# squellww/super-resolution-system

Measured on AMD Instinct MI355X. Metric: megapixels/sec tile+blend+QA at 200MP, 1/2/4/8 GPU, higher is better.
Workload: dtype f32; 1 GPU; 720p->200MP 17320x11550 canvas, 25 tiles 4124x2970, 6-level Laplacian blend (cosine weights) + PSNR + SSIM(uniform7,gauss11,simple); tile_pixels=306207000, canvas_pixels=200046000, parallelism=single, stream=assessment of image i on a second HIP stream beside tile+pyramids of image i+1

## Files before the change

include/sr_hip.h:

```cpp
#ifndef SR_HIP_H
#define SR_HIP_H

#include <stddef.h>
#include <stdint.h>

#ifdef __cplusplus
extern "C" {
#endif

#define SR_API __attribute__((visibility("default")))

enum sr_status {
    SR_OK = 0,
    SR_ERR_INVALID_ARG = -1,
    SR_ERR_SHAPE = -2,
    SR_ERR_OOM = -3,
    SR_ERR_HIP = -4,
    SR_ERR_COMM = -5,
    SR_ERR_UNSUPPORTED = -6
};

enum sr_pad_mode { SR_PAD_MIRROR = 0, SR_PAD_REPLICATE = 1, SR_PAD_REFLECT = 2, SR_PAD_CONSTANT = 3 };
enum sr_weight_type { SR_W_LINEAR = 0, SR_W_COSINE = 1, SR_W_SIGMOID = 2,
                      SR_W_ONES = 3 };
// ... 212 lines not shown
    double ssim_simple;
} sr_assess_sums;
SR_API int sr_assess_u8_async(sr_ctx *ctx, const uint8_t *d_a, int64_t stride_a, const uint8_t *d_b,
                              int64_t stride_b, int h, int w, int cn, int gray_shift, double data_range,
                              int row_begin, int row_end, int flags, sr_assess_sums *d_out);
SR_API int sr_assess_u8(sr_ctx *ctx, const uint8_t *d_a, int64_t stride_a, const uint8_t *d_b,
                        int64_t stride_b, int h, int w, int cn, int gray_shift, double data_range,
                        int row_begin, int row_end, int flags, sr_assess_sums *h_out);
SR_API int sr_assess_resized_u8_async(sr_ctx *ctx, const uint8_t *d_a, int64_t stride_a, const uint8_t *d_b,
                                      int64_t stride_b, int h, int w, int cn, int dst_h, int dst_w,
                                      int gray_shift, double data_range, int flags, sr_assess_sums *d_out);
SR_API int sr_assess_resized_u8(sr_ctx *ctx, const uint8_t *d_a, int64_t stride_a, const uint8_t *d_b,
                                int64_t stride_b, int h, int w, int cn, int dst_h, int dst_w, int gray_shift,
                                double data_range, int flags, sr_assess_sums *h_out);
SR_API int sr_ssim_count(int h, int w, int mode, int row_begin, int row_end, uint64_t *count);
typedef struct sr_quality_cell {
    uint64_t sse;
    double ssim_uniform;
    double ssim_gauss;
    double ssim_simple;
} sr_quality_cell;
SR_API int sr_quality_map_u8(sr_ctx *ctx, const uint8_t *d_a, int64_t stride_a, const uint8_t *d_b, int64_t stride_b,
                             int h, int w, int cn, int gray_shift, double data_range, const int *h_xedges, int gw,
                             const int *h_yedges, int gh, int flags, sr_quality_cell *h_out);
SR_API int sr_quality_map_counts(int h, int w, int mode, const int *h_xedges, int gw, const int *h_yedges, int gh,
                                 uint64_t *counts);
typedef struct sr_ms_ssim_level {
    double sum_lcs;
    double sum_cs;
    uint64_t count;
// ... 381 lines not shown
```

super-resolution-system_amd/_native.py:

```python
from __future__ import annotations

import ctypes as C
import math
import os
import threading
from typing import List, Optional, Sequence, Tuple

import numpy as np

_HERE = os.path.dirname(os.path.abspath(__file__))
LIB_PATH = os.environ.get("SR_LIB_PATH") or os.path.join(_HERE, "libsrhip.so")

SR_OK = 0
SR_ERR_INVALID_ARG, SR_ERR_SHAPE, SR_ERR_OOM, SR_ERR_HIP, SR_ERR_COMM, SR_ERR_UNSUPPORTED = -1, -2, -3, -4, -5, -6
PAD_MODES = {"mirror": 0, "replicate": 1, "reflect": 2, "constant": 3}
WEIGHT_TYPES = {"linear": 0, "cosine": 1, "sigmoid": 2, "ones": 3}
SSIM_MODES = {"uniform": 0, "gauss": 1, "simple": 2}
SR_U8, SR_F32, SR_F64 = 0, 1, 2
POISSON_MAX_SIDE = 16385


class SrNativeError(RuntimeError):
    """HIP / library failure (SR_ERR_HIP, SR_ERR_OOM, SR_ERR_COMM, SR_ERR_UNSUPPORTED)."""

# ... 238 lines not shown
    "sr_sse_u8": (_i, [_vp, _vp, _i64, _vp, _i64, _i, _i64, C.POINTER(C.c_uint64)]),
    "sr_sse_u8_async": (_i, [_vp, _vp, _i64, _vp, _i64, _i, _i64, _vp]),
    "sr_psnr_from_sse": (_dbl, [C.c_uint64, C.c_uint64, _dbl]),
    "sr_seam_scan": (_i, [_vp, _vp, _i64, _i, _i, _i, C.POINTER(TileRect), C.POINTER(_vp), C.POINTER(_i64), _i, _i, _i, _i,
                          _dbl, C.POINTER(SeamRecord), _i, _pi]),
    "sr_sse_f32": (_i, [_vp, _vp, _i64, _vp, _i64, _i, _i64, C.POINTER(_dbl)]),
    "sr_weighted_blend_custom": (_i, [_vp, _i, C.POINTER(_vp), C.POINTER(_i64), C.POINTER(_vp), C.POINTER(_i64), _vp, _i64, _vp]),
    "sr_ssim_u8": (_i, [_vp, _vp, _i64, _vp, _i64, _i, _i, _i, _i, _i, _dbl, _i, _i, C.POINTER(_dbl), C.POINTER(C.c_uint64)]),
    "sr_ssim_float": (_i, [_vp, _i, _vp, _i64, _vp, _i64, _i, _i, _i, _i, _dbl, _i, _i, C.POINTER(_dbl), C.POINTER(C.c_uint64)]),
    "sr_ssim_u8_async": (_i, [_vp, _vp, _i64, _vp, _i64, _i, _i, _i, _i, _i, _dbl, _i, _i, _vp, C.POINTER(C.c_uint64)]),
    "sr_assess_u8_async": (_i, [_vp, _vp, _i64, _vp, _i64, _i, _i, _i, _i, _dbl, _i, _i, _i, _vp]),
    "sr_assess_u8": (_i, [_vp, _vp, _i64, _vp, _i64, _i, _i, _i, _i, _dbl, _i, _i, _i, C.POINTER(AssessSums)]),
    "sr_assess_resized_u8_async": (_i, [_vp, _vp, _i64, _vp, _i64, _i, _i, _i, _i, _i, _i, _dbl, _i, _vp]),
    "sr_assess_resized_u8": (_i, [_vp, _vp, _i64, _vp, _i64, _i, _i, _i, _i, _i, _i, _dbl, _i, C.POINTER(AssessSums)]),
    "sr_ssim_count": (_i, [_i, _i, _i, _i, _i, C.POINTER(C.c_uint64)]),
    "sr_quality_map_u8": (_i, [_vp, _vp, _i64, _vp, _i64, _i, _i, _i, _i, _dbl, _pi, _i, _pi, _i, _i, C.POINTER(QualityCell)]),
    "sr_quality_map_counts": (_i, [_i, _i, _i, _pi, _i, _pi, _i, C.POINTER(C.c_uint64)]),
    "sr_ms_ssim_plan": (_i, [_i, _i, _i, _pi, _pi, C.POINTER(C.c_uint64), C.POINTER(_sz)]),
    "sr_ms_ssim_u8": (_i, [_vp, _vp, _i64, _vp, _i64, _i, _i, _i, _i, _dbl, _i, C.POINTER(MsSsimLevel)]),
    "sr_ms_ssim_value": (_dbl, [C.POINTER(MsSsimLevel), _i, C.POINTER(_dbl)]),
    "sr_ms_ssim_planes": (_i, [_vp, _i, _vp, _vp]),
    "sr_bench_plan": (_i, [_i, _i, _i, _i, _i, _pi, _pi, C.POINTER(C.c_uint64), C.POINTER(C.c_uint64), C.POINTER(_sz)]),
    "sr_bench_u8": (_i, [_vp, _vp, _i64, _vp, _i64, _i, _i, _i, _i, _i, _dbl, C.POINTER(BenchSums)]),
    "sr_vif_plan": (_i, [_i, _i, _i, _i, _i, _pi, _pi, C.POINTER(C.c_uint64), C.POINTER(_sz)]),
    "sr_vif_window": (_i, [_i, C.POINTER(_dbl)]),
    "sr_vif_u8": (_i, [_vp, _vp, _i64, _vp, _i64, _i, _i, _i, _i, _i, C.POINTER(VifScale)]),
    "sr_vif_value": (_dbl, [C.POINTER(VifScale), _i]),
    "sr_gmsd_plan": (_i, [_i, _i, _i, _i, _i, _pi, _pi, C.POINTER(C.c_uint64), C.POINTER(_sz)]),
    "sr_gmsd_u8": (_i, [_vp, _vp, _i64, _vp, _i64, _i, _i, _i, _i, _i, C.POINTER(GmsdSums)]),
    "sr_gmsd_value": (_dbl, [C.POINTER(GmsdSums)]),
# ... 329 lines not shown


def color_table_class(glut: np.ndarray, terms: int = 64) -> int:
    g = np.ascontiguousarray(glut, dtype=np.float32).reshape(-1, 256)
    cls = C.c_int(-1)
    check(load().sr_color_table_class(g.ctypes.data_as(C.POINTER(C.c_float)), int(g.shape[0]), int(terms), C.byref(cls)))
    return cls.value


def ssim_count(h: int, w: int, mode: str, row_begin: int = 0, row_end: Optional[int] = None) -> int:
    n = C.c_uint64(0)
    check(load().sr_ssim_count(h, w, SSIM_MODES[mode], row_begin, h if row_end is None else row_end, C.byref(n)))
    return n.value


def _edge_array(edges, name: str):
    e = np.asarray(edges)
    if e.ndim != 1 or e.size < 2 or e.dtype.kind not in "iu":
        raise ValueError(f"{name}: need a flat list of at least two integer edges")
    if e.min() < -2 ** 31 or e.max() >= 2 ** 31:
        raise ValueError(f"{name}: edge out of range")
    return (C.c_int * e.size)(*[int(v) for v in e]), int(e.size) - 1


def quality_map_counts(h: int, w: int, mode: str, x_edges, y_edges) -> np.ndarray:
    xe, gw = _edge_array(x_edges, "x_edges")
    ye, gh = _edge_array(y_edges, "y_edges")
    out = np.zeros((gh, gw), dtype=np.uint64)
    check(load().sr_quality_map_counts(int(h), int(w), SSIM_MODES[mode], xe, gw, ye, gh,
                                       out.ctypes.data_as(C.POINTER(C.c_uint64))))
# ... 2187 lines not shown
```

super-resolution-system_amd/csrc/sr_assess.hip:

```cpp
#include <hip/hip_runtime.h>

#include <algorithm>
#include <cmath>
#include <cstdlib>
#include <cstring>
#include <mutex>
#include <set>
#include <vector>

#include "sr_ctx.h"
#include "sr_device.h"
#include "sr_ssim11.h"

__device__ __forceinline__ unsigned long long wave_sum_u64(unsigned long long v)
{
#pragma unroll
    for (int o = 32; o > 0; o >>= 1) v += __shfl_down(v, o, 64);
    return v;
}

__device__ __forceinline__ double wave_sum_f64(double v)
{
#pragma unroll
    for (int o = 32; o > 0; o >>= 1) v += __shfl_down(v, o, 64);
    return v;
}

__global__ __launch_bounds__(256) void k_sse_flat(const uint4 *__restrict__ a, const uint4 *__restrict__ b,
                                                  size_t nvec, const unsigned char *__restrict__ ta,
                                                  const unsigned char *__restrict__ tb, int ntail,
                                                  unsigned long long *__restrict__ out)
{
    unsigned long long s = 0;
    const size_t stride = (size_t)gridDim.x * blockDim.x;
    for (size_t i = (size_t)blockIdx.x * blockDim.x + threadIdx.x; i < nvec; i += stride) {
        const uint4 va = a[i], vb = b[i];
        const unsigned int wa[4] = {va.x, va.y, va.z, va.w}, wb[4] = {vb.x, vb.y, vb.z, vb.w};
        unsigned int p = 0;
#pragma unroll
        for (int k = 0; k < 4; ++k)
#pragma unroll
            for (int j = 0; j < 4; ++j) {
// ... 68 lines not shown
{
    const int x = blockIdx.x * 64 + threadIdx.x, y = blockIdx.y * 4 + threadIdx.y;
    if (x >= w || y >= h) return;
    gray[(size_t)y * gstride + x] = (unsigned char)gray_of(rgb + (size_t)y * stride + (size_t)x * 3, 3, shift);
}

struct CubicTab {
    int ofs;
    short c[4];
};

enum { ASSESS_SSE = 1, ASSESS_UNIFORM = 2, ASSESS_GAUSS = 4, ASSESS_SIMPLE = 8, ASSESS_ALL_BITS = 15 };

struct AssessParams {
    int h, w, shift, ry0, ry1, flags, same_c;
    int nch, ty;
    double c1a, c2a;
    double c1b, c2b;
    double k1u, k2u;
    double k[6];
};

template <int CN>
__device__ __forceinline__ void load_gray_pair(const unsigned char *__restrict__ a, long long sa,
                                               const unsigned char *__restrict__ b, long long sb, int sy, int sx,
                                               int shift, int &ga, int &gb, unsigned &sq)
{
    const unsigned char *pa = a + (size_t)sy * sa + (size_t)sx * CN;
    const unsigned char *pb = b + (size_t)sy * sb + (size_t)sx * CN;
    gray_pair<CN>(pa, pb, shift, ga, gb, sq);
}


__device__ __forceinline__ double fast_recip(double d)
{
// ... 50 lines not shown
        for (int c = 0; c < CN; ++c) {
            const int hs = v[0][c] * X.c[0] + v[1][c] * X.c[1] + v[2][c] * X.c[2] + v[3][c] * X.c[3];
            acc[c] += hs * (int)yc[ky];
        }
    }
#pragma unroll
    for (int c = 0; c < CN; ++c) {
        const int t = (acc[c] + (1 << 21)) >> 22;
        out[c] = t < 0 ? 0 : (t > 255 ? 255 : t);
    }
}

template <int CN>
__device__ __forceinline__ unsigned assess_load_chunk(const unsigned char *__restrict__ a, long long sa,
                                                      const unsigned char *__restrict__ b, long long sb,
                                                      const AssessParams &P, int bx0, int by0, int ch,
                                                      int rows_needed, unsigned (*XY)[AM_GP],
                                                      unsigned (*QQ)[AM_GP], unsigned (*PP)[AM_GP])
{
    unsigned sse = 0;
    const bool want_sse = (P.flags & ASSESS_SSE) != 0;
    for (int i = threadIdx.x; i < AM_CH * (AM_GP / 4); i += AM_TX) {
        const int ly = i / (AM_GP / 4), lx = (i - ly * (AM_GP / 4)) * 4;
        const int lr = ch * AM_CH + ly;
        if (lr >= rows_needed) break;
        const int gy = by0 - AM_R + lr, gx = bx0 - AM_R + lx;
        const int sy = reflect101(gy, P.h);
        int ga[4], gb[4];
        unsigned sq[4];
        if (gx >= 0 && gx + 3 < P.w) {
            const unsigned char *pa = a + (size_t)sy * sa + (size_t)gx * CN;
            const unsigned char *pb = b + (size_t)sy * sb + (size_t)gx * CN;
            if (CN == 3) {
                const u3_t qa = ld_u3_a1(pa), qb = ld_u3_a1(pb);
                const unsigned wa[3] = {qa.x, qa.y, qa.z}, wb[3] = {qb.x, qb.y, qb.z};
                int ca[12], cb[12];
#pragma unroll
// ... 24 lines not shown
        }
        u4_t vxy, vq, vp;
        unsigned txy[4], tq[4], tp[4];
#pragma unroll
        for (int k = 0; k < 4; ++k) {
            txy[k] = (unsigned)ga[k] | ((unsigned)gb[k] << 14);
            tq[k] = (unsigned)__mul24(ga[k], gb[k]);
            tp[k] = (unsigned)(__mul24(ga[k], ga[k]) + __mul24(gb[k], gb[k]));
        }
        vxy.x = txy[0]; vxy.y = txy[1]; vxy.z = txy[2]; vxy.w = txy[3];
        vq.x = tq[0]; vq.y = tq[1]; vq.z = tq[2]; vq.w = tq[3];
        vp.x = tp[0]; vp.y = tp[1]; vp.z = tp[2]; vp.w = tp[3];
        *(u4_t *)&XY[ly][lx] = vxy;
        *(u4_t *)&QQ[ly][lx] = vq;
        *(u4_t *)&PP[ly][lx] = vp;
        if (want_sse && lr >= AM_R && lr < AM_R + P.ty && gy < P.ry1 && gy < P.h) {
#pragma unroll
            for (int k = 0; k < 4; ++k)
                if (lx + k >= AM_R && lx + k < AM_R + AM_TX && gx + k < P.w) sse += sq[k];
        }
    }
    return sse;
}

typedef __attribute__((address_space(3))) const unsigned lds_cu32;
__device__ __forceinline__ lds_cu32 *lds_row_base(lds_cu32 *row0, int bytes)
{
    lds_cu32 *q;
    asm volatile("v_add_u32 %0, %2, %1" : "=v"(q) : "v"(row0), "n"(bytes));
    return q;
}

template <int CN, bool GAUSS, bool UNIF, bool SAMEC>
__global__ __launch_bounds__(AM_TX, 3) void k_assess_march(const unsigned char *__restrict__ a, long long sa,
                                                      const unsigned char *__restrict__ b, long long sb,
                                                      AssessParams P, double *__restrict__ part)
{
    __shared__ __attribute__((aligned(16))) unsigned L3[3][AM_CH][AM_GP];
    unsigned (*XY)[AM_GP] = L3[0];
    unsigned (*QQ)[AM_GP] = L3[1];
    unsigned (*PP)[AM_GP] = L3[2];
    __shared__ unsigned U[UNIF ? 7 : 1][2][AM_TX];
    __shared__ double red[AM_TX / 64][4];
    const int c = threadIdx.x;
    const int bx0 = blockIdx.x * AM_TX, by0 = P.ry0 + blockIdx.y * P.ty;
    const int rows_needed = min(P.ty, P.ry1 - by0) + 2 * AM_R;
    const int mx = bx0 + c;
    double f[GAUSS ? 4 : 1][11];
    if (GAUSS) {
#pragma unroll
        for (int m = 0; m < 4; ++m)
#pragma unroll
            for (int i = 0; i < 11; ++i) f[m][i] = 0.0;
    }
    unsigned t_xy = 0, t_p = 0, t_q = 0;
    double sum_int = 0.0, sum_all = 0.0, sum_u = 0.0;
    unsigned sse = 0;
    int slot = 0;
    const double k0 = P.k[0], k1 = P.k[1], k2 = P.k[2], k3 = P.k[3], k4 = P.k[4], k5 = P.k[5];
    lds_cu32 *xy0 = (lds_cu32 *)&L3[0][0][c];
    constexpr int MAPB = AM_CH * AM_GP * 4;
    __shared__ double EDGE[(GAUSS && SAMEC) ? AM_TX : 1];
    if (GAUSS && SAMEC) EDGE[c] = 0.0;
#pragma unroll 1
    for (int ch = 0; ch < P.nch; ++ch) {
        if (ch * AM_CH >= rows_needed) break;
        __syncthreads();
        sse += assess_load_chunk<CN>(a, sa, b, sb, P, bx0, by0, ch, rows_needed, XY, QQ, PP);
        __syncthreads();
#pragma unroll
        for (int s = 0; s < AM_CH; ++s) {
            const int r = ch * AM_CH + s;
            if (r >= rows_needed) continue;
            lds_cu32 *rxy = lds_row_base(xy0, s * AM_GP * 4), *rq = lds_row_base(xy0, MAPB + s * AM_GP * 4),
                     *rp = lds_row_base(xy0, 2 * MAPB + s * AM_GP * 4);
            unsigned xy[11], qv[11], pv[11];
#pragma unroll
            for (int j = 0; j < 11; ++j) {
                xy[j] = rxy[j];
                qv[j] = rq[j];
                pv[j] = rp[j];
            }
            unsigned sxy[6], sp[6], sq[6];
            sxy[0] = xy[5]; sp[0] = pv[5]; sq[0] = qv[5];
#pragma unroll
            for (int j = 1; j <= (GAUSS ? AM_R : 3); ++j) {
                sxy[j] = xy[5 - j] + xy[5 + j];
                sp[j] = pv[5 - j] + pv[5 + j];
                sq[j] = qv[5 - j] + qv[5 + j];
            }
            if (GAUSS) {
                const double kk[6] = {k0, k1, k2, k3, k4, k5};
                double hx = (double)(sxy[0] & 0x3FFFu) * kk[0], hy = (double)(sxy[0] >> 14) * kk[0];
                double hp = (double)sp[0] * kk[0], hq = (double)sq[0] * kk[0];
#pragma unroll
                for (int j = 1; j <= AM_R; ++j) {
                    hx = fma((double)(sxy[j] & 0x3FFFu), kk[j], hx);
                    hy = fma((double)(sxy[j] >> 14), kk[j], hy);
                    hp = fma((double)sp[j], kk[j], hp);
                    hq = fma((double)sq[j], kk[j], hq);
                }
                f[0][s] = hx; f[1][s] = hy; f[2][s] = hp; f[3][s] = hq;
            }
            if (UNIF) {
                const unsigned uxy = ((sxy[0] + sxy[1]) + sxy[2]) + sxy[3];
                const unsigned up = ((sp[0] + sp[1]) + sp[2]) + sp[3];
                const unsigned uq = ((sq[0] + sq[1]) + sq[2]) + sq[3];
                if (r >= 7) {
                    const unsigned o0 = U[slot][0][c], o1 = U[slot][1][c];
                    t_xy -= o0 & 0x1FFFFFFu;
                    t_p -= o1 & 0xFFFFFu;
                    t_q -= (o0 >> 25) | ((o1 >> 20) << 7);
                }
                t_xy += uxy; t_p += up; t_q += uq;
                U[slot][0][c] = uxy | (uq << 25);
                U[slot][1][c] = up | ((uq >> 7) << 20);
                slot = slot == 6 ? 0 : slot + 1;
                const int orow = r - 8, my = by0 + orow;
                if (orow >= 0 && orow < P.ty && my < P.ry1 && my >= 3 && my < P.h - 3) {
                    const int sx = (int)(t_xy & 0x3FFFu), sy = (int)(t_xy >> 14);
                    const int sxsy = __mul24(sx, sy), ss = __mul24(sx, sx) + __mul24(sy, sy);
                    const int ncov = __mul24(49, (int)t_q) - sxsy, nvar = __mul24(49, (int)t_p) - ss;
                    const double a1 = fma(2.0, (double)sxsy, P.k1u), a2 = fma(2.0, (double)ncov, P.k2u);
                    const double b1 = (double)ss + P.k1u, b2 = (double)nvar + P.k2u;
                    sum_u += (a1 * a2) * ssim_recip(b1 * b2);
                }
            }
            if (GAUSS && r >= 2 * AM_R) {
                const int orow = r - 2 * AM_R, my = by0 + orow;
                if (orow < P.ty && my < P.ry1 && my < P.h) {
                    const double kk[6] = {k0, k1, k2, k3, k4, k5};
                    double u[4];
#pragma unroll
                    for (int m = 0; m < 4; ++m) {
                        double acc = f[m][(s + 6) % 11] * kk[0];
#pragma unroll
                        for (int j = 1; j <= AM_R; ++j)
                            acc = fma(f[m][(s + 6 + 11 - j) % 11] + f[m][(s + 6 + j) % 11], kk[j], acc);
                        u[m] = acc;
                    }
                    const bool inner_row = my >= AM_R && my < P.h - AM_R;
                    if (SAMEC) {
                        const double sv = ssim_quot(u[0], u[1], u[2], u[3], P.c1a, P.c2a);
                        sum_all += sv;
                        if (!inner_row) EDGE[c] += sv;
                    } else {
                        if (P.flags & ASSESS_SIMPLE) sum_all += ssim_quot(u[0], u[1], u[2], u[3], P.c1b, P.c2b);
                        if (inner_row && (P.flags & ASSESS_GAUSS)) sum_int += ssim_quot(u[0], u[1], u[2], u[3], P.c1a, P.c2a);
                    }
                }
            }
        }
    }
    if (GAUSS && SAMEC) sum_int = sum_all - EDGE[c];
    if (!(mx < P.w)) sum_all = 0.0;
    if (!(mx >= AM_R && mx < P.w - AM_R)) sum_int = 0.0;
    if (!(mx >= 3 && mx < P.w - 3)) sum_u = 0.0;
    sum_int = wave_sum_f64(sum_int);
    sum_all = wave_sum_f64(sum_all);
    sum_u = wave_sum_f64(sum_u);
    const double dsse = wave_sum_f64((double)sse);
    if ((c & 63) == 0) {
        red[c >> 6][0] = sum_int;
        red[c >> 6][1] = sum_all;
        red[c >> 6][2] = dsse;
        red[c >> 6][3] = sum_u;
    }
    __syncthreads();
    if (c < 4) {
        const size_t blk = (size_t)blockIdx.y * gridDim.x + blockIdx.x;
        double t = red[0][c];
#pragma unroll
        for (int wv = 1; wv < AM_TX / 64; ++wv) t += red[wv][c];
        part[blk * 4 + c] = t;
    }
}

__global__ __launch_bounds__(256) void k_reduce_partials(const double *__restrict__ part, long long n, int ncomp,
                                                         double *__restrict__ out)
{
    __shared__ double sh[256];
    const long long base = (long long)blockIdx.x * 1024;
    for (int comp = 0; comp < ncomp; ++comp) {
        double s = 0.0;
        for (int k = 0; k < 4; ++k) {
            const long long i = base + k * 256 + threadIdx.x;
            if (i < n) s += part[i * ncomp + comp];
        }
        sh[threadIdx.x] = s;
// ... 463 lines not shown
            }
        }
    }
    const double sred = wave_sum_f64((double)sse);
    if ((tid & 63) == 0) ws[tid >> 6] = sred;
    __syncthreads();
    if (tid == 0) part[(size_t)blockIdx.y * gridDim.x + blockIdx.x] = (ws[0] + ws[1]) + (ws[2] + ws[3]);
}

__global__ void k_store_sse(const double *__restrict__ src, sr_assess_sums *__restrict__ out)
{
    if (threadIdx.x == 0 && blockIdx.x == 0) out->sse = src[0];
}

__global__ __launch_bounds__(256) void k_assess_finish(const double *__restrict__ part, long long n, int flags,
                                                       sr_assess_sums *__restrict__ out)
{
    __shared__ double sh[4][256];
    double s[4] = {0.0, 0.0, 0.0, 0.0};
    for (long long i = threadIdx.x; i < n; i += 256) {
#pragma unroll
        for (int c = 0; c < 4; ++c) s[c] += part[i * 4 + c];
    }
#pragma unroll
    for (int c = 0; c < 4; ++c) sh[c][threadIdx.x] = s[c];
    __syncthreads();
    for (int o = 128; o > 0; o >>= 1) {
        if ((int)threadIdx.x < o) {
#pragma unroll
            for (int c = 0; c < 4; ++c) sh[c][threadIdx.x] += sh[c][threadIdx.x + o];
        }
        __syncthreads();
    }
    if (threadIdx.x == 0) {
        out->ssim_gauss = (flags & ASSESS_GAUSS) ? sh[0][0] : 0.0;
        out->ssim_simple = (flags & ASSESS_SIMPLE) ? sh[1][0] : 0.0;
        out->sse = (flags & ASSESS_SSE) ? sh[2][0] : 0.0;
        out->ssim_uniform = (flags & ASSESS_UNIFORM) ? sh[3][0] : 0.0;
    }
}

__global__ void k_assess_store(const double *__restrict__ g, const double *__restrict__ u, int flags,
                               sr_assess_sums *__restrict__ out)
{
    if (threadIdx.x != 0 || blockIdx.x != 0) return;
    out->ssim_gauss = (g && (flags & ASSESS_GAUSS)) ? g[0] : 0.0;
    out->ssim_simple = (g && (flags & ASSESS_SIMPLE)) ? g[1] : 0.0;
    out->sse = (g && (flags & ASSESS_SSE)) ? g[2] : 0.0;
    out->ssim_uniform = (u && (flags & ASSESS_UNIFORM)) ? u[0] : 0.0;
// ... 167 lines not shown
    HIPCHK(hipMemcpyAsync(h_sse, scr, sizeof(uint64_t), hipMemcpyDeviceToHost, ctx->stream));
    HIPCHK(stream_sync(ctx));
    return SR_OK;
}

int sr_ssim_count(int h, int w, int mode, int row_begin, int row_end, uint64_t *count)
{
    if (!count || h < 1 || w < 1) return sr_set_error(SR_ERR_INVALID_ARG, "sr_ssim_count: bad arguments");
    int pad;
    if (mode == SR_SSIM_UNIFORM7) pad = 3;
    else if (mode == SR_SSIM_GAUSS11) pad = 5;
    else if (mode == SR_SSIM_SIMPLE) pad = 0;
    else return sr_set_error(SR_ERR_INVALID_ARG, "sr_ssim_count: unknown mode %d", mode);
    const long long y0 = std::max(pad, row_begin), y1 = std::min(h - pad, row_end), nx = (long long)w - 2 * pad;
    *count = (y1 > y0 && nx > 0) ? (uint64_t)((y1 - y0) * nx) : 0;
    return SR_OK;
}

static int assess_impl(sr_ctx *ctx, const uint8_t *d_a, int64_t stride_a, const uint8_t *d_b, int64_t stride_b, int h,
                       int w, int cn, int gray_shift, double data_range, int row_begin, int row_end, int flags,
                       sr_assess_sums *d_out, const char *scope)
{
    if (!d_a || !d_b || !d_out) return sr_set_error(SR_ERR_INVALID_ARG, "%s: null argument", scope);
    if (h < 1 || w < 1 || (cn != 1 && cn != 3)) return sr_set_error(SR_ERR_INVALID_ARG, "%s: need h,w >= 1 and 1 or 3 channels", scope);
    if (gray_shift != 14 && gray_shift != 15) return sr_set_error(SR_ERR_INVALID_ARG, "%s: gray_shift must be 14 or 15", scope);
    const int64_t min_stride = (int64_t)w * cn;
    if (stride_a < min_stride || stride_b < min_stride) return sr_set_error(SR_ERR_SHAPE, "%s: stride smaller than a row", scope);
    row_begin = std::max(row_begin, 0);
    row_end = std::min(row_end, h);
    AssessParams P;
    memset(&P, 0, sizeof(P));
    P.h = h; P.w = w; P.shift = gray_shift; P.ry0 = row_begin; P.ry1 = row_end; P.flags = flags;
    P.c1a = (0.01 * data_range) * (0.01 * data_range);
    P.c2a = (0.03 * data_range) * (0.03 * data_range);
    P.c1b = (0.01 * 255.0) * (0.01 * 255.0);
    P.c2b = (0.03 * 255.0) * (0.03 * 255.0);
    P.same_c = (P.c1a == P.c1b && P.c2a == P.c2b) ? 1 : 0;
    P.k1u = 2401.0 * P.c1a;
    P.k2u = 2352.0 * P.c2a;
    gauss_taps(P.k);
    const int rows = row_end - row_begin;
    if (rows > 0 && (flags & ASSESS_ALL_BITS)) {
        const long long gbx = (w + AM_TX - 1) / AM_TX;
        const long long slots = (long long)std::max(ctx->num_cu, 1) * 3;
        long long best_cost = -1;
        for (int n = 2; n <= AM_NCH_MAX; ++n) {
            const int ty = AM_CH * n - 2 * AM_R;
            const long long blocks = gbx * ((rows + ty - 1) / ty);
            const long long cost = ((blocks + slots - 1) / slots) * (AM_CH * n);
            if (best_cost < 0 || cost <= best_cost) { best_cost = cost; P.nch = n; P.ty = ty; }
        }
        if (const char *e = std::getenv("SR_ASSESS_NCH")) {
            char *end = nullptr;
            const long n = std::strtol(e, &end, 10);
            if (end != e && *end == '\0' && n >= 2 && n <= AM_NCH_MAX) { P.nch = (int)n; P.ty = AM_CH * (int)n - 2 * AM_R; }
        }
        const long long gby = (rows + P.ty - 1) / P.ty;
        const size_t nblk = (size_t)(gbx * gby);
        void *scr = nullptr;
        int rc = ctx_scratch(ctx, std::max<size_t>(nblk * 4 * 8 + 512, (size_t)8 << 20), &scr);
        if (rc) return rc;
        double *part = (double *)scr;
        {
            ProfScope ps(ctx, scope);
            const dim3 grid((unsigned)gbx, (unsigned)gby), block(AM_TX);
#define LAUNCH_ASSESS(CNV, GS, US, SC)                                                                               \
    hipLaunchKernelGGL((k_assess_march<CNV, GS, US, SC>), grid, block, 0, ctx->stream, d_a, (long long)stride_a, d_b,   \
                       (long long)stride_b, P, part)
#define LAUNCH_ASSESS_V(CNV)                                                                                            \
    do {                                                                                                                \
        if (gauss && unif) { if (P.same_c) LAUNCH_ASSESS(CNV, true, true, true); else LAUNCH_ASSESS(CNV, true, true, false); } \
        else if (gauss) { if (P.same_c) LAUNCH_ASSESS(CNV, true, false, true); else LAUNCH_ASSESS(CNV, true, false, false); } \
        else if (unif) LAUNCH_ASSESS(CNV, false, true, true);                                                           \
        else LAUNCH_ASSESS(CNV, false, false, true);                                                                    \
    } while (0)
            const bool gauss = (flags & (ASSESS_GAUSS | ASSESS_SIMPLE)) != 0, unif = (flags & ASSESS_UNIFORM) != 0;
            if (cn == 3) LAUNCH_ASSESS_V(3);
            else LAUNCH_ASSESS_V(1);
#undef LAUNCH_ASSESS_V
#undef LAUNCH_ASSESS
            hipLaunchKernelGGL(k_assess_finish, dim3(1), dim3(256), 0, ctx->stream, part, (long long)nblk, flags, d_out);
        }
        return check_launch("assess");
    }
    hipLaunchKernelGGL(k_assess_store, dim3(1), dim3(64), 0, ctx->stream, (const double *)nullptr, (const double *)nullptr, flags, d_out);
    return check_launch("assess");
}

int sr_assess_u8_async(sr_ctx *ctx, const uint8_t *d_a, int64_t stride_a, const uint8_t *d_b, int64_t stride_b, int h,
                       int w, int cn, int gray_shift, double data_range, int row_begin, int row_end, int flags,
                       sr_assess_sums *d_out)
{
    CTX_ENTER(ctx);
    return assess_impl(ctx, d_a, stride_a, d_b, stride_b, h, w, cn, gray_shift, data_range, row_begin, row_end, flags,
                       d_out, "assess_all");
}
// ... 271 lines not shown
```

super-resolution-system_amd/csrc/sr_ctx.h:

```cpp
#pragma once
#include <hip/hip_runtime.h>

#include <mutex>
#include <string>
#include <vector>

#include "sr_internal.h"

#define SRCHK(expr)                                                                                \
    do {                                                                                           \
        const int rc_ = (expr);                                                                    \
        if (rc_ != SR_OK) return rc_;                                                              \
    } while (0)

#define HIPCHK(expr)                                                                               \
    do {                                                                                           \
        hipError_t e_ = (expr);                                                                    \
        if (e_ != hipSuccess)                                                                      \
            return sr_set_error(SR_ERR_HIP, "%s: %s (%s:%d)", #expr, hipGetErrorString(e_), __FILE__, \
                                __LINE__);                                                         \
    } while (0)

struct sr_ctx;

// ... 60 lines not shown
    DevBuf niqe_ws;
    int niqe_H = 0, niqe_W = 0;
    DevBuf brisque_ws;
    int brisque_H2 = 0, brisque_W2 = 0;
    DevBuf vif_ws;
    DevBuf gmsd_ws;
    DevBuf fsim_ws;
    int fsim_rows = 0, fsim_cols = 0;
    double fsim_consts[12] = {0};
    DevBuf vsi_ws;
    int vsi_h = 0, vsi_w = 0;
    DevBuf deltae_ws;
    bool deltae_table = false;
    DevBuf haarpsi_ws;
    CachedTable imresize_tab;
    void release_device()
    {
        for (DevBuf *b : {&scratch, &extract_tab.buf, &resize_tab.buf, &cubic_tab.buf, &gray_planes, &cm_ws, &msssim_ws, &bench_ws, &niqe_ws, &brisque_ws, &vif_ws, &gmsd_ws, &fsim_ws, &vsi_ws, &deltae_ws, &haarpsi_ws, &imresize_tab.buf})
            b->release();
    }
};

hipError_t upload_small(sr_ctx *c, void *d_dst, const void *h_src, size_t bytes);
hipError_t stream_sync(sr_ctx *c);
hipError_t upload_if_changed(sr_ctx *c, void *d_dst, const void *h_src, size_t bytes, std::vector<char> &shadow);
int upload_cached(sr_ctx *c, CachedTable &t, const void *h_src, size_t bytes);
bool ctx_is_live(const sr_ctx *c);
struct sr_blend_plan;
bool plan_describe(const sr_blend_plan *p, sr_ctx **ctx, int *n, int *cn);
void destroy_plans_of(sr_ctx *ctx);
int ctx_scratch(sr_ctx *c, size_t bytes, void **out);
hipEvent_t prof_event(sr_ctx *c);
int check_launch(const char *what);
// ... 53 lines not shown
```

Baseline: 68740 MP/s.

## Drive assess kernel from a device work-item list with optional persistent blocks

```diff
diff --git a/include/sr_hip.h b/include/sr_hip.h
--- a/include/sr_hip.h
+++ b/include/sr_hip.h
@@ -250,6 +250,7 @@
                                 int64_t stride_b, int h, int w, int cn, int dst_h, int dst_w, int gray_shift,
                                 double data_range, int flags, sr_assess_sums *h_out);
 SR_API int sr_ssim_count(int h, int w, int mode, int row_begin, int row_end, uint64_t *count);
+SR_API int sr_assess_plan_items(int w, int row_begin, int row_end, int num_cu, int32_t *out, int64_t cap, int64_t *count);
 typedef struct sr_quality_cell {
     uint64_t sse;
     double ssim_uniform;
diff --git a/super-resolution-system_amd/_native.py b/super-resolution-system_amd/_native.py
--- a/super-resolution-system_amd/_native.py
+++ b/super-resolution-system_amd/_native.py
@@ -276,6 +276,7 @@
     "sr_assess_resized_u8_async": (_i, [_vp, _vp, _i64, _vp, _i64, _i, _i, _i, _i, _i, _i, _dbl, _i, _vp]),
     "sr_assess_resized_u8": (_i, [_vp, _vp, _i64, _vp, _i64, _i, _i, _i, _i, _i, _i, _dbl, _i, C.POINTER(AssessSums)]),
     "sr_ssim_count": (_i, [_i, _i, _i, _i, _i, C.POINTER(C.c_uint64)]),
+    "sr_assess_plan_items": (_i, [_i, _i, _i, _i, C.POINTER(C.c_int32), _i64, C.POINTER(_i64)]),
     "sr_quality_map_u8": (_i, [_vp, _vp, _i64, _vp, _i64, _i, _i, _i, _i, _dbl, _pi, _i, _pi, _i, _i, C.POINTER(QualityCell)]),
     "sr_quality_map_counts": (_i, [_i, _i, _i, _pi, _i, _pi, _i, C.POINTER(C.c_uint64)]),
     "sr_ms_ssim_plan": (_i, [_i, _i, _i, _pi, _pi, C.POINTER(C.c_uint64), C.POINTER(_sz)]),
@@ -635,6 +636,15 @@
     return n.value
 
 
+def assess_plan_items(w: int, row_begin: int, row_end: int, num_cu: int) -> np.ndarray:
+    cnt = C.c_int64(0)
+    check(load().sr_assess_plan_items(int(w), int(row_begin), int(row_end), int(num_cu), None, 0, C.byref(cnt)))
+    out = np.zeros((cnt.value, 4), np.int32)
+    check(load().sr_assess_plan_items(int(w), int(row_begin), int(row_end), int(num_cu),
+                                      out.ctypes.data_as(C.POINTER(C.c_int32)), cnt.value, C.byref(cnt)))
+    return out
+
+
 def _edge_array(edges, name: str):
     e = np.asarray(edges)
     if e.ndim != 1 or e.size < 2 or e.dtype.kind not in "iu":
diff --git a/super-resolution-system_amd/csrc/sr_assess.hip b/super-resolution-system_amd/csrc/sr_assess.hip
--- a/super-resolution-system_amd/csrc/sr_assess.hip
+++ b/super-resolution-system_amd/csrc/sr_assess.hip
@@ -26,6 +26,17 @@
     return v;
 }
 
+__device__ __forceinline__ double wave_sum_f64_lane(double v, int lane)
+{
+#pragma unroll
+    for (int o = 32; o > 0; o >>= 1) {
+        const int src = (lane + o) << 2;
+        const int lo = __builtin_amdgcn_ds_bpermute(src, __double2loint(v)), hi = __builtin_amdgcn_ds_bpermute(src, __double2hiint(v));
+        v += __hiloint2double(hi, lo);
+    }
+    return v;
+}
+
 __global__ __launch_bounds__(256) void k_sse_flat(const uint4 *__restrict__ a, const uint4 *__restrict__ b,
                                                   size_t nvec, const unsigned char *__restrict__ ta,
                                                   const unsigned char *__restrict__ tb, int ntail,
@@ -124,11 +135,14 @@
 
 struct AssessParams {
     int h, w, shift, ry0, ry1, flags, same_c;
-    int nch, ty;
     double c1a, c2a;
     double c1b, c2b;
     double k1u, k2u;
     double k[6];
+};
+
+struct AssessItem {
+    int bx0, by0, nch, index;
 };
 
 template <int CN>
@@ -209,13 +223,13 @@
 template <int CN>
 __device__ __forceinline__ unsigned assess_load_chunk(const unsigned char *__restrict__ a, long long sa,
                                                       const unsigned char *__restrict__ b, long long sb,
-                                                      const AssessParams &P, int bx0, int by0, int ch,
+                                                      const AssessParams &P, int tid, int bx0, int by0, int ty, int ch,
                                                       int rows_needed, unsigned (*XY)[AM_GP],
                                                       unsigned (*QQ)[AM_GP], unsigned (*PP)[AM_GP])
 {
     unsigned sse = 0;
     const bool want_sse = (P.flags & ASSESS_SSE) != 0;
-    for (int i = threadIdx.x; i < AM_CH * (AM_GP / 4); i += AM_TX) {
+    for (int i = tid; i < AM_CH * (AM_GP / 4); i += AM_TX) {
         const int ly = i / (AM_GP / 4), lx = (i - ly * (AM_GP / 4)) * 4;
         const int lr = ch * AM_CH + ly;
         if (lr >= rows_needed) break;
@@ -270,7 +284,7 @@
         *(u4_t *)&XY[ly][lx] = vxy;
         *(u4_t *)&QQ[ly][lx] = vq;
         *(u4_t *)&PP[ly][lx] = vp;
-        if (want_sse && lr >= AM_R && lr < AM_R + P.ty && gy < P.ry1 && gy < P.h) {
+        if (want_sse && lr >= AM_R && lr < AM_R + ty && gy < P.ry1 && gy < P.h) {
 #pragma unroll
             for (int k = 0; k < 4; ++k)
                 if (lx + k >= AM_R && lx + k < AM_R + AM_TX && gx + k < P.w) sse += sq[k];
@@ -290,7 +304,9 @@
 template <int CN, bool GAUSS, bool UNIF, bool SAMEC>
 __global__ __launch_bounds__(AM_TX, 3) void k_assess_march(const unsigned char *__restrict__ a, long long sa,
                                                       const unsigned char *__restrict__ b, long long sb,
-                                                      AssessParams P, double *__restrict__ part)
+                                                      AssessParams P, const AssessItem *__restrict__ items,
+                                                      int n_items, unsigned *__restrict__ counter,
+                                                      double *__restrict__ part)
 {
     __shared__ __attribute__((aligned(16))) unsigned L3[3][AM_CH][AM_GP];
     unsigned (*XY)[AM_GP] = L3[0];
@@ -298,137 +314,155 @@
     unsigned (*PP)[AM_GP] = L3[2];
     __shared__ unsigned U[UNIF ? 7 : 1][2][AM_TX];
     __shared__ double red[AM_TX / 64][4];
-    const int c = threadIdx.x;
-    const int bx0 = blockIdx.x * AM_TX, by0 = P.ry0 + blockIdx.y * P.ty;
-    const int rows_needed = min(P.ty, P.ry1 - by0) + 2 * AM_R;
-    const int mx = bx0 + c;
-    double f[GAUSS ? 4 : 1][11];
-    if (GAUSS) {
-#pragma unroll
-        for (int m = 0; m < 4; ++m)
-#pragma unroll
-            for (int i = 0; i < 11; ++i) f[m][i] = 0.0;
-    }
-    unsigned t_xy = 0, t_p = 0, t_q = 0;
-    double sum_int = 0.0, sum_all = 0.0, sum_u = 0.0;
-    unsigned sse = 0;
-    int slot = 0;
-    const double k0 = P.k[0], k1 = P.k[1], k2 = P.k[2], k3 = P.k[3], k4 = P.k[4], k5 = P.k[5];
-    lds_cu32 *xy0 = (lds_cu32 *)&L3[0][0][c];
+    __shared__ unsigned claim;
     constexpr int MAPB = AM_CH * AM_GP * 4;
     __shared__ double EDGE[(GAUSS && SAMEC) ? AM_TX : 1];
-    if (GAUSS && SAMEC) EDGE[c] = 0.0;
+    int c = threadIdx.x;
 #pragma unroll 1
-    for (int ch = 0; ch < P.nch; ++ch) {
-        if (ch * AM_CH >= rows_needed) break;
-        __syncthreads();
-        sse += assess_load_chunk<CN>(a, sa, b, sb, P, bx0, by0, ch, rows_needed, XY, QQ, PP);
-        __syncthreads();
-#pragma unroll
-        for (int s = 0; s < AM_CH; ++s) {
-            const int r = ch * AM_CH + s;
-            if (r >= rows_needed) continue;
-            lds_cu32 *rxy = lds_row_base(xy0, s * AM_GP * 4), *rq = lds_row_base(xy0, MAPB + s * AM_GP * 4),
-                     *rp = lds_row_base(xy0, 2 * MAPB + s * AM_GP * 4);
-            unsigned xy[11], qv[11], pv[11];
-#pragma unroll
-            for (int j = 0; j < 11; ++j) {
-                xy[j] = rxy[j];
-                qv[j] = rq[j];
-                pv[j] = rp[j];
-            }
-            unsigned sxy[6], sp[6], sq[6];
-            sxy[0] = xy[5]; sp[0] = pv[5]; sq[0] = qv[5];
-#pragma unroll
-            for (int j = 1; j <= (GAUSS ? AM_R : 3); ++j) {
-                sxy[j] = xy[5 - j] + xy[5 + j];
-                sp[j] = pv[5 - j] + pv[5 + j];
-                sq[j] = qv[5 - j] + qv[5 + j];
-            }
-            if (GAUSS) {
-                const double kk[6] = {k0, k1, k2, k3, k4, k5};
-                double hx = (double)(sxy[0] & 0x3FFFu) * kk[0], hy = (double)(sxy[0] >> 14) * kk[0];
-                double hp = (double)sp[0] * kk[0], hq = (double)sq[0] * kk[0];
-#pragma unroll
-                for (int j = 1; j <= AM_R; ++j) {
-                    hx = fma((double)(sxy[j] & 0x3FFFu), kk[j], hx);
-                    hy = fma((double)(sxy[j] >> 14), kk[j], hy);
-                    hp = fma((double)sp[j], kk[j], hp);
-                    hq = fma((double)sq[j], kk[j], hq);
+    for (;;) {
+        asm volatile("" : "+v"(c));
+        int it = blockIdx.x;
+        if (counter) {
+            if (c == 0) claim = atomicAdd(counter, 1u);
+            __syncthreads();
+            it = __builtin_amdgcn_readfirstlane((int)claim);
+        }
+        if (it >= n_items) break;
+        const int bx0 = __builtin_amdgcn_readfirstlane(items[it].bx0), by0 = __builtin_amdgcn_readfirstlane(items[it].by0);
+        const int nch = __builtin_amdgcn_readfirstlane(items[it].nch), index = __builtin_amdgcn_readfirstlane(items[it].index);
+        const int ty = AM_CH * nch - 2 * AM_R;
+        const int rows_needed = min(ty, P.ry1 - by0) + 2 * AM_R;
+        const int mx = bx0 + c;
+        const double k0 = P.k[0], k1 = P.k[1], k2 = P.k[2], k3 = P.k[3], k4 = P.k[4], k5 = P.k[5];
+        lds_cu32 *xy0 = (lds_cu32 *)&L3[0][0][c];
+        double f[GAUSS ? 4 : 1][11];
+        if (GAUSS) {
+#pragma unroll
+            for (int m = 0; m < 4; ++m)
+#pragma unroll
+                for (int i = 0; i < 11; ++i) f[m][i] = 0.0;
+        }
+        unsigned t_xy = 0, t_p = 0, t_q = 0;
+        double sum_int = 0.0, sum_all = 0.0, sum_u = 0.0;
+        unsigned sse = 0;
+        int slot = 0;
+        if (GAUSS && SAMEC) {
+            double zero = 0.0;
+            asm volatile("" : "+v"(zero));
+            EDGE[c] = zero;
+        }
+#pragma unroll 1
+        for (int ch = 0; ch < nch; ++ch) {
+            if (ch * AM_CH >= rows_needed) break;
+            __syncthreads();
+            sse += assess_load_chunk<CN>(a, sa, b, sb, P, c, bx0, by0, ty, ch, rows_needed, XY, QQ, PP);
+            __syncthreads();
+#pragma unroll
+            for (int s = 0; s < AM_CH; ++s) {
+                const int r = ch * AM_CH + s;
+                if (r >= rows_needed) continue;
+                lds_cu32 *rxy = lds_row_base(xy0, s * AM_GP * 4), *rq = lds_row_base(xy0, MAPB + s * AM_GP * 4),
+                         *rp = lds_row_base(xy0, 2 * MAPB + s * AM_GP * 4);
+                unsigned xy[11], qv[11], pv[11];
+#pragma unroll
+                for (int j = 0; j < 11; ++j) {
+                    xy[j] = rxy[j];
+                    qv[j] = rq[j];
+                    pv[j] = rp[j];
                 }
-                f[0][s] = hx; f[1][s] = hy; f[2][s] = hp; f[3][s] = hq;
-            }
-            if (UNIF) {
-                const unsigned uxy = ((sxy[0] + sxy[1]) + sxy[2]) + sxy[3];
-                const unsigned up = ((sp[0] + sp[1]) + sp[2]) + sp[3];
-                const unsigned uq = ((sq[0] + sq[1]) + sq[2]) + sq[3];
-                if (r >= 7) {
-                    const unsigned o0 = U[slot][0][c], o1 = U[slot][1][c];
-                    t_xy -= o0 & 0x1FFFFFFu;
-                    t_p -= o1 & 0xFFFFFu;
-                    t_q -= (o0 >> 25) | ((o1 >> 20) << 7);
+                unsigned sxy[6], sp[6], sq[6];
+                sxy[0] = xy[5]; sp[0] = pv[5]; sq[0] = qv[5];
+#pragma unroll
+                for (int j = 1; j <= (GAUSS ? AM_R : 3); ++j) {
+                    sxy[j] = xy[5 - j] + xy[5 + j];
+                    sp[j] = pv[5 - j] + pv[5 + j];
+                    sq[j] = qv[5 - j] + qv[5 + j];
                 }
-                t_xy += uxy; t_p += up; t_q += uq;
-                U[slot][0][c] = uxy | (uq << 25);
-                U[slot][1][c] = up | ((uq >> 7) << 20);
-                slot = slot == 6 ? 0 : slot + 1;
-                const int orow = r - 8, my = by0 + orow;
-                if (orow >= 0 && orow < P.ty && my < P.ry1 && my >= 3 && my < P.h - 3) {
-                    const int sx = (int)(t_xy & 0x3FFFu), sy = (int)(t_xy >> 14);
-                    const int sxsy = __mul24(sx, sy), ss = __mul24(sx, sx) + __mul24(sy, sy);
-                    const int ncov = __mul24(49, (int)t_q) - sxsy, nvar = __mul24(49, (int)t_p) - ss;
-                    const double a1 = fma(2.0, (double)sxsy, P.k1u), a2 = fma(2.0, (double)ncov, P.k2u);
-                    const double b1 = (double)ss + P.k1u, b2 = (double)nvar + P.k2u;
-                    sum_u += (a1 * a2) * ssim_recip(b1 * b2);
+                if (GAUSS) {
+                    const double kk[6] = {k0, k1, k2, k3, k4, k5};
+                    double hx = (double)(sxy[0] & 0x3FFFu) * kk[0], hy = (double)(sxy[0] >> 14) * kk[0];
+                    double hp = (double)sp[0] * kk[0], hq = (double)sq[0] * kk[0];
+#pragma unroll
+                    for (int j = 1; j <= AM_R; ++j) {
+                        hx = fma((double)(sxy[j] & 0x3FFFu), kk[j], hx);
+                        hy = fma((double)(sxy[j] >> 14), kk[j], hy);
+                        hp = fma((double)sp[j], kk[j], hp);
+                        hq = fma((double)sq[j], kk[j], hq);
+                    }
+                    f[0][s] = hx; f[1][s] = hy; f[2][s] = hp; f[3][s] = hq;
                 }
-            }
-            if (GAUSS && r >= 2 * AM_R) {
-                const int orow = r - 2 * AM_R, my = by0 + orow;
-                if (orow < P.ty && my < P.ry1 && my < P.h) {
-                    const double kk[6] = {k0, k1, k2, k3, k4, k5};
-                    double u[4];
-#pragma unroll
-                    for (int m = 0; m < 4; ++m) {
-                        double acc = f[m][(s + 6) % 11] * kk[0];
-#pragma unroll
-                        for (int j = 1; j <= AM_R; ++j)
-                            acc = fma(f[m][(s + 6 + 11 - j) % 11] + f[m][(s + 6 + j) % 11], kk[j], acc);
-                        u[m] = acc;
+                if (UNIF) {
+                    const unsigned uxy = ((sxy[0] + sxy[1]) + sxy[2]) + sxy[3];
+                    const unsigned up = ((sp[0] + sp[1]) + sp[2]) + sp[3];
+                    const unsigned uq = ((sq[0] + sq[1]) + sq[2]) + sq[3];
+                    if (r >= 7) {
+                        const unsigned o0 = U[slot][0][c], o1 = U[slot][1][c];
+                        t_xy -= o0 & 0x1FFFFFFu;
+                        t_p -= o1 & 0xFFFFFu;
+                        t_q -= (o0 >> 25) | ((o1 >> 20) << 7);
                     }
-                    const bool inner_row = my >= AM_R && my < P.h - AM_R;
-                    if (SAMEC) {
-                        const double sv = ssim_quot(u[0], u[1], u[2], u[3], P.c1a, P.c2a);
-                        sum_all += sv;
-                        if (!inner_row) EDGE[c] += sv;
-                    } else {
-                        if (P.flags & ASSESS_SIMPLE) sum_all += ssim_quot(u[0], u[1], u[2], u[3], P.c1b, P.c2b);
-                        if (inner_row && (P.flags & ASSESS_GAUSS)) sum_int += ssim_quot(u[0], u[1], u[2], u[3], P.c1a, P.c2a);
+                    t_xy += uxy; t_p += up; t_q += uq;
+                    U[slot][0][c] = uxy | (uq << 25);
+                    U[slot][1][c] = up | ((uq >> 7) << 20);
+                    slot = slot == 6 ? 0 : slot + 1;
+                    const int orow = r - 8, my = by0 + orow;
+                    if (orow >= 0 && orow < ty && my < P.ry1 && my >= 3 && my < P.h - 3) {
+                        const int sx = (int)(t_xy & 0x3FFFu), sy = (int)(t_xy >> 14);
+                        const int sxsy = __mul24(sx, sy), ss = __mul24(sx, sx) + __mul24(sy, sy);
+                        const int ncov = __mul24(49, (int)t_q) - sxsy, nvar = __mul24(49, (int)t_p) - ss;
+                        const double a1 = fma(2.0, (double)sxsy, P.k1u), a2 = fma(2.0, (double)ncov, P.k2u);
+                        const double b1 = (double)ss + P.k1u, b2 = (double)nvar + P.k2u;
+                        sum_u += (a1 * a2) * ssim_recip(b1 * b2);
                     }
                 }
-            }
-        }
-    }
-    if (GAUSS && SAMEC) sum_int = sum_all - EDGE[c];
-    if (!(mx < P.w)) sum_all = 0.0;
-    if (!(mx >= AM_R && mx < P.w - AM_R)) sum_int = 0.0;
-    if (!(mx >= 3 && mx < P.w - 3)) sum_u = 0.0;
-    sum_int = wave_sum_f64(sum_int);
-    sum_all = wave_sum_f64(sum_all);
-    sum_u = wave_sum_f64(sum_u);
-    const double dsse = wave_sum_f64((double)sse);
-    if ((c & 63) == 0) {
-        red[c >> 6][0] = sum_int;
-        red[c >> 6][1] = sum_all;
-        red[c >> 6][2] = dsse;
-        red[c >> 6][3] = sum_u;
-    }
-    __syncthreads();
-    if (c < 4) {
-        const size_t blk = (size_t)blockIdx.y * gridDim.x + blockIdx.x;
-        double t = red[0][c];
-#pragma unroll
-        for (int wv = 1; wv < AM_TX / 64; ++wv) t += red[wv][c];
-        part[blk * 4 + c] = t;
+                if (GAUSS && r >= 2 * AM_R) {
+                    const int orow = r - 2 * AM_R, my = by0 + orow;
+                    if (orow < ty && my < P.ry1 && my < P.h) {
+                        const double kk[6] = {k0, k1, k2, k3, k4, k5};
+                        double u[4];
+#pragma unroll
+                        for (int m = 0; m < 4; ++m) {
+                            double acc = f[m][(s + 6) % 11] * kk[0];
+#pragma unroll
+                            for (int j = 1; j <= AM_R; ++j)
+                                acc = fma(f[m][(s + 6 + 11 - j) % 11] + f[m][(s + 6 + j) % 11], kk[j], acc);
+                            u[m] = acc;
+                        }
+                        const bool inner_row = my >= AM_R && my < P.h - AM_R;
+                        if (SAMEC) {
+                            const double sv = ssim_quot(u[0], u[1], u[2], u[3], P.c1a, P.c2a);
+                            sum_all += sv;
+                            if (!inner_row) EDGE[c] += sv;
+                        } else {
+                            if (P.flags & ASSESS_SIMPLE) sum_all += ssim_quot(u[0], u[1], u[2], u[3], P.c1b, P.c2b);
+                            if (inner_row && (P.flags & ASSESS_GAUSS)) sum_int += ssim_quot(u[0], u[1], u[2], u[3], P.c1a, P.c2a);
+                        }
+                    }
+                }
+            }
+        }
+        if (GAUSS && SAMEC) sum_int = sum_all - EDGE[c];
+        if (!(mx < P.w)) sum_all = 0.0;
+        if (!(mx >= AM_R && mx < P.w - AM_R)) sum_int = 0.0;
+        if (!(mx >= 3 && mx < P.w - 3)) sum_u = 0.0;
+        sum_int = wave_sum_f64_lane(sum_int, c & 63);
+        sum_all = wave_sum_f64_lane(sum_all, c & 63);
+        sum_u = wave_sum_f64_lane(sum_u, c & 63);
+        const double dsse = wave_sum_f64_lane((double)sse, c & 63);
+        if ((c & 63) == 0) {
+            red[c >> 6][0] = sum_int;
+            red[c >> 6][1] = sum_all;
+            red[c >> 6][2] = dsse;
+            red[c >> 6][3] = sum_u;
+        }
+        __syncthreads();
+        if (c < 4) {
+            double t = red[0][c];
+#pragma unroll
+            for (int wv = 1; wv < AM_TX / 64; ++wv) t += red[wv][c];
+            part[(size_t)index * 4 + c] = t;
+        }
+        if (!counter) break;
     }
 }
 
@@ -922,7 +956,7 @@
 }
 
 __global__ __launch_bounds__(256) void k_assess_finish(const double *__restrict__ part, long long n, int flags,
-                                                       sr_assess_sums *__restrict__ out)
+                                                       unsigned *__restrict__ counter, sr_assess_sums *__restrict__ out)
 {
     __shared__ double sh[4][256];
     double s[4] = {0.0, 0.0, 0.0, 0.0};
@@ -941,6 +975,7 @@
         __syncthreads();
     }
     if (threadIdx.x == 0) {
+        if (counter) *counter = 0;
         out->ssim_gauss = (flags & ASSESS_GAUSS) ? sh[0][0] : 0.0;
         out->ssim_simple = (flags & ASSESS_SIMPLE) ? sh[1][0] : 0.0;
         out->sse = (flags & ASSESS_SSE) ? sh[2][0] : 0.0;
@@ -1138,6 +1173,54 @@
     else return sr_set_error(SR_ERR_INVALID_ARG, "sr_ssim_count: unknown mode %d", mode);
     const long long y0 = std::max(pad, row_begin), y1 = std::min(h - pad, row_end), nx = (long long)w - 2 * pad;
     *count = (y1 > y0 && nx > 0) ? (uint64_t)((y1 - y0) * nx) : 0;
+    return SR_OK;
+}
+
+static bool env_int_in(const char *name, long lo, long hi, int *out)
+{
+    const char *e = std::getenv(name);
+    if (!e) return false;
+    char *end = nullptr;
+    const long n = std::strtol(e, &end, 10);
+    if (end == e || *end != '\0' || n < lo || n > hi) return false;
+    *out = (int)n;
+    return true;
+}
+
+static int assess_uniform_nch(int w, int rows, int num_cu)
+{
+    const long long gbx = (w + AM_TX - 1) / AM_TX, slots = (long long)std::max(num_cu, 1) * 3;
+    long long best_cost = -1;
+    int nch = 2;
+    for (int n = 2; n <= AM_NCH_MAX; ++n) {
+        const int ty = AM_CH * n - 2 * AM_R;
+        const long long blocks = gbx * ((rows + ty - 1) / ty);
+        const long long cost = ((blocks + slots - 1) / slots) * (AM_CH * n);
+        if (best_cost < 0 || cost <= best_cost) { best_cost = cost; nch = n; }
+    }
+    (void)env_int_in("SR_ASSESS_NCH", 2, AM_NCH_MAX, &nch);
+    return nch;
+}
+
+static void assess_items_uniform(int w, int ry0, int ry1, int nch, std::vector<AssessItem> &items)
+{
+    const int gbx = (w + AM_TX - 1) / AM_TX, ty = AM_CH * nch - 2 * AM_R, gby = (ry1 - ry0 + ty - 1) / ty;
+    items.clear();
+    items.reserve((size_t)gbx * gby);
+    for (int by = 0; by < gby; ++by)
+        for (int bx = 0; bx < gbx; ++bx) items.push_back({bx * AM_TX, ry0 + by * ty, nch, by * gbx + bx});
+}
+
+int sr_assess_plan_items(int w, int row_begin, int row_end, int num_cu, int32_t *out, int64_t cap, int64_t *count)
+{
+    if (!count || w < 1 || row_end <= row_begin || num_cu < 1) return sr_set_error(SR_ERR_INVALID_ARG, "sr_assess_plan_items: bad arguments");
+    std::vector<AssessItem> items;
+    assess_items_uniform(w, row_begin, row_end, assess_uniform_nch(w, row_end - row_begin, num_cu), items);
+    *count = (int64_t)items.size();
+    if (out) {
+        if (cap < *count) return sr_set_error(SR_ERR_INVALID_ARG, "sr_assess_plan_items: %lld items, room for %lld", (long long)*count, (long long)cap);
+        memcpy(out, items.data(), items.size() * sizeof(AssessItem));
+    }
     return SR_OK;
 }
 
@@ -1165,32 +1248,29 @@
     gauss_taps(P.k);
     const int rows = row_end - row_begin;
     if (rows > 0 && (flags & ASSESS_ALL_BITS)) {
-        const long long gbx = (w + AM_TX - 1) / AM_TX;
-        const long long slots = (long long)std::max(ctx->num_cu, 1) * 3;
-        long long best_cost = -1;
-        for (int n = 2; n <= AM_NCH_MAX; ++n) {
-            const int ty = AM_CH * n - 2 * AM_R;
-            const long long blocks = gbx * ((rows + ty - 1) / ty);
-            const long long cost = ((blocks + slots - 1) / slots) * (AM_CH * n);
-            if (best_cost < 0 || cost <= best_cost) { best_cost = cost; P.nch = n; P.ty = ty; }
-        }
-        if (const char *e = std::getenv("SR_ASSESS_NCH")) {
-            char *end = nullptr;
-            const long n = std::strtol(e, &end, 10);
-            if (end != e && *end == '\0' && n >= 2 && n <= AM_NCH_MAX) { P.nch = (int)n; P.ty = AM_CH * (int)n - 2 * AM_R; }
-        }
-        const long long gby = (rows + P.ty - 1) / P.ty;
-        const size_t nblk = (size_t)(gbx * gby);
+        std::vector<AssessItem> items;
+        assess_items_uniform(w, row_begin, row_end, assess_uniform_nch(w, rows, ctx->num_cu), items);
+        const size_t nblk = items.size();
+        SRCHK(upload_cached(ctx, ctx->assess_items, items.data(), nblk * sizeof(AssessItem)));
+        int nblocks = 0;
+        const bool persistent = env_int_in("SR_ASSESS_BLOCKS", 1, 3 * std::max(ctx->num_cu, 1), &nblocks);
+        nblocks = persistent ? (int)std::min<size_t>((size_t)nblocks, nblk) : (int)nblk;
+        if (persistent && !ctx->assess_counter.d) {
+            SRCHK(ctx->assess_counter.reserve(ctx, scope, 256));
+            HIPCHK(hipMemsetAsync(ctx->assess_counter.d, 0, 256, ctx->stream));
+        }
         void *scr = nullptr;
         int rc = ctx_scratch(ctx, std::max<size_t>(nblk * 4 * 8 + 512, (size_t)8 << 20), &scr);
         if (rc) return rc;
         double *part = (double *)scr;
         {
             ProfScope ps(ctx, scope);
-            const dim3 grid((unsigned)gbx, (unsigned)gby), block(AM_TX);
+            const dim3 grid((unsigned)nblocks), block(AM_TX);
+            const AssessItem *d_items = ctx->assess_items.buf.as<const AssessItem>();
+            unsigned *d_counter = persistent ? ctx->assess_counter.as<unsigned>() : nullptr;
 #define LAUNCH_ASSESS(CNV, GS, US, SC)                                                                               \
     hipLaunchKernelGGL((k_assess_march<CNV, GS, US, SC>), grid, block, 0, ctx->stream, d_a, (long long)stride_a, d_b,   \
-                       (long long)stride_b, P, part)
+                       (long long)stride_b, P, d_items, (int)nblk, d_counter, part)
 #define LAUNCH_ASSESS_V(CNV)                                                                                            \
     do {                                                                                                                \
         if (gauss && unif) { if (P.same_c) LAUNCH_ASSESS(CNV, true, true, true); else LAUNCH_ASSESS(CNV, true, true, false); } \
@@ -1203,7 +1283,7 @@
             else LAUNCH_ASSESS_V(1);
 #undef LAUNCH_ASSESS_V
 #undef LAUNCH_ASSESS
-            hipLaunchKernelGGL(k_assess_finish, dim3(1), dim3(256), 0, ctx->stream, part, (long long)nblk, flags, d_out);
+            hipLaunchKernelGGL(k_assess_finish, dim3(1), dim3(256), 0, ctx->stream, part, (long long)nblk, flags, d_counter, d_out);
         }
         return check_launch("assess");
     }
diff --git a/super-resolution-system_amd/csrc/sr_ctx.h b/super-resolution-system_amd/csrc/sr_ctx.h
--- a/super-resolution-system_amd/csrc/sr_ctx.h
+++ b/super-resolution-system_amd/csrc/sr_ctx.h
@@ -98,9 +98,11 @@
     bool deltae_table = false;
     DevBuf haarpsi_ws;
     CachedTable imresize_tab;
+    CachedTable assess_items;
+    DevBuf assess_counter;
     void release_device()
     {
-        for (DevBuf *b : {&scratch, &extract_tab.buf, &resize_tab.buf, &cubic_tab.buf, &gray_planes, &cm_ws, &msssim_ws, &bench_ws, &niqe_ws, &brisque_ws, &vif_ws, &gmsd_ws, &fsim_ws, &vsi_ws, &deltae_ws, &haarpsi_ws, &imresize_tab.buf})
+        for (DevBuf *b : {&scratch, &extract_tab.buf, &resize_tab.buf, &cubic_tab.buf, &gray_planes, &cm_ws, &msssim_ws, &bench_ws, &niqe_ws, &brisque_ws, &vif_ws, &gmsd_ws, &fsim_ws, &vsi_ws, &deltae_ws, &haarpsi_ws, &imresize_tab.buf, &assess_items.buf, &assess_counter})
             b->release();
     }
 };
```

Measured after the change: 68470 MP/s. About the same (-0.4%).
